# fluhus/frackyfrac

Measured on NVIDIA B200. Metric: UniFrac sample-pairs/sec (unweighted), higher is better.
Workload: dtype u8 x u8 -> s32 (tcgen05 kind::i8, exact), s64 chunk / row sums, f32 ratio / output

## Files before the change

### frackyfrac_b200/csrc/embed.cu

```cuda
#include "frc_internal.h"

namespace frc {

namespace {

constexpr int kThreads = 256;

__global__ void k_scatter_f64(const int64_t* __restrict__ row_ptr, const int32_t* __restrict__ col,
                              const double* __restrict__ val, int64_t s_base, int64_t s_end, double* E,
                              int64_t ld, int32_t* __restrict__ K, int32_t kp) {
  int64_t s = s_base + ((static_cast<int64_t>(blockIdx.x) * blockDim.x + threadIdx.x) >> 5);
  int lane = threadIdx.x & 31;
  if (s >= s_end) return;
  int64_t b = row_ptr[s], e = row_ptr[s + 1];
  for (int64_t k = b + lane; k < e; k += 32) {
    E[static_cast<int64_t>(col[k]) * ld + (s - s_base)] = val[k];
    if (K) K[((s >> 7) * kp + col[k]) * 128 + (s & 127)] = col[k];
  }
}

__global__ void k_level_sum_f64(const int32_t* __restrict__ nodes, const int32_t* __restrict__ child_ptr,
                                const int32_t* __restrict__ child_idx, double* E, int64_t ld,
                                int32_t* __restrict__ K, int32_t kp, int64_t s_base) {
  int32_t v = nodes[blockIdx.x];
// ... 170 lines not shown
  const int32_t v0 = blockIdx.x * 64;
  const int32_t w0 = blockIdx.y * 8;
  for (int idx = threadIdx.x; idx < 512; idx += 256) {
    int node = idx >> 3, word = idx & 7;
    uint32_t x = 0;
    if (v0 + node < n_nodes && w0 + word < nw)
      x = bits[static_cast<int64_t>(v0 + node) * nw + w0 + word];
    words[node][word] = x;
  }
  __syncthreads();
  const int wi = threadIdx.x >> 5, lane = threadIdx.x & 31;
  const int32_t va = v0 + 2 * lane, vb = va + 1;
  const uint32_t wa = words[2 * lane][wi], wb = words[2 * lane + 1][wi];
  const uint32_t ha = va < n_nodes ? len_hi[va] : 0, hb = vb < n_nodes ? len_hi[vb] : 0;
  const uint32_t la = va < n_nodes ? len_lo[va] : 0, lb = vb < n_nodes ? len_lo[vb] : 0;
  const int64_t s0 = (static_cast<int64_t>(w0) + wi) * 32;
#pragma unroll 4
  for (int it = 0; it < 32; ++it) {
    const int64_t s = s0 + it;
    if (s >= np) break;
    const uint32_t ba = (wa >> it) & 1u, bb = (wb >> it) & 1u;
    const int64_t o = s * kp + va;
    const uint32_t ma = 0u - ba, mb = 0u - bb;
    *reinterpret_cast<uint32_t*>(P + o) = (0x3F80u & ma) | ((0x3F80u & mb) << 16);
    *reinterpret_cast<uint32_t*>(Bh + o) = (ha & ma) | ((hb & mb) << 16);
    *reinterpret_cast<uint32_t*>(Bl + o) = (la & ma) | ((lb & mb) << 16);
  }
}


template <bool kSmem>
__global__ void __launch_bounds__(512)
k_embed_presence_fused(const int64_t* __restrict__ row_ptr, const int32_t* __restrict__ col,
                       int64_t n_samples, const int32_t* __restrict__ level_nodes,
                       const int32_t* __restrict__ level_parent, const int32_t* __restrict__ level_ptr,
                       int32_t height, int32_t n_nodes, int32_t kp, const int32_t* __restrict__ order,
                       uint32_t* __restrict__ node_scratch, uint32_t* __restrict__ bitsT, int32_t w0,
                       uint32_t* __restrict__ bitsS, const PeerPtrs peers) {
  extern __shared__ __align__(16) uint32_t smem_words[];
  __shared__ int32_t lptr[128];
  const int w = blockIdx.x + w0;
  const int tid = threadIdx.x, lane = tid & 31, warp = tid >> 5;
  uint32_t* colw = kSmem ? smem_words : node_scratch + static_cast<int64_t>(blockIdx.x) * n_nodes;

  for (int32_t v = tid; v < n_nodes; v += 512) colw[v] = 0u;
  if (tid < 128 && tid <= height + 1) lptr[tid] = level_ptr[tid];
  __syncthreads();
  {
    int64_t rb[2], re[2];
#pragma unroll
    for (int u = 0; u < 2; ++u) {
      const int64_t s = static_cast<int64_t>(w) * 32 + warp + 16 * u;
      rb[u] = s < n_samples ? row_ptr[s] : 0;
      re[u] = s < n_samples ? row_ptr[s + 1] : 0;
    }
#pragma unroll
    for (int u = 0; u < 2; ++u) {
      const uint32_t bit = 1u << (warp + 16 * u);
      for (int64_t k = rb[u] + lane; k < re[u]; k += 256) {
        int32_t c[8];
#pragma unroll
        for (int x = 0; x < 8; ++x) c[x] = k + 32 * x < re[u] ? col[k + 32 * x] : -1;
#pragma unroll
        for (int x = 0; x < 8; ++x)
          if (c[x] >= 0) atomicOr(colw + c[x], bit);
      }
    }
  }
  __syncthreads();
  auto lp = [&](int32_t h) { return h < 128 ? lptr[h] : level_ptr[h]; };
  int32_t h = 0;
  for (; h < height; ++h) {
    const int32_t b = lp(h), e = lp(h + 1);
    if (e - b <= 512) break;
    for (int32_t idx = b + tid; idx < e; idx += 4096) {
      int32_t n[8], p[8];
#pragma unroll
      for (int u = 0; u < 8; ++u) {
        const int32_t k = idx + u * 512;
        n[u] = k < e ? level_nodes[k] : -1;
        p[u] = k < e ? level_parent[k] : 0;
      }
#pragma unroll
      for (int u = 0; u < 8; ++u)
        if (n[u] >= 0) {
          const uint32_t x = colw[n[u]];
          if (x) atomicOr(colw + p[u], x);
        }
    }
    __syncthreads();
  }
  for (; h < height; h += 8) {
    int32_t n[8], p[8];
#pragma unroll
    for (int u = 0; u < 8; ++u) {
      n[u] = -1; p[u] = 0;
      if (h + u < height) {
        const int32_t k = lp(h + u) + tid;
        if (k < lp(h + u + 1)) { n[u] = level_nodes[k]; p[u] = level_parent[k]; }
      }
    }
#pragma unroll
    for (int u = 0; u < 8; ++u) {
      if (h + u < height) {
        if (n[u] >= 0) {
          const uint32_t x = colw[n[u]];
          if (x) atomicOr(colw + p[u], x);
        }
        __syncthreads();
      }
    }
  }
  uint32_t* dst = bitsT + static_cast<int64_t>(w) * kp;
  if (peers.n > 0) {
    const int64_t at = static_cast<int64_t>(w) * kp;
#pragma unroll 4
    for (int32_t k = tid; k < kp; k += 512) {
      const int32_t v = order[k];
      const uint32_t x = v >= 0 ? colw[v] : 0u;
#pragma unroll
      for (int pr = 0; pr < 8; ++pr)
        if (pr < peers.n) peers.p[pr][at + k] = x;
    }
  } else {
#pragma unroll 8
    for (int32_t k = tid; k < kp; k += 512) {
      const int32_t v = order[k];
      dst[k] = v >= 0 ? colw[v] : 0u;
    }
  }
  if (bitsS != nullptr) {
    const int32_t words = kp >> 5;
    for (int32_t g = warp; g * 128 < kp; g += 16) {
      uint32_t wout[4];
#pragma unroll
      for (int u = 0; u < 4; ++u) {
        const int32_t v = order[g * 128 + u * 32 + lane];
        const uint32_t wv = v >= 0 ? colw[v] : 0u;
        uint32_t mine = 0;
// ... 318 lines not shown
    ++launches;
  }
  return launches;
}

int launch_presence_rowsum(const uint32_t* bits, int32_t n_nodes, int32_t nw, const double* lenq,
                           double* r, double* scratch, cudaStream_t s) {
  int chunks = pick_chunks(n_nodes);
  dim3 grid(nw, chunks);
  k_presence_rowsum<<<grid, 32, 0, s>>>(bits, n_nodes, nw, lenq, scratch);
  int64_t ld = static_cast<int64_t>(nw) * 32;
  k_reduce_partials<<<static_cast<unsigned>((ld + kThreads - 1) / kThreads), kThreads, 0, s>>>(
      scratch, chunks, ld, ld, r);
  return 2;
}

int launch_expand_operands(const uint32_t* bits, int32_t n_nodes, int32_t nw, int32_t kp, int64_t np,
                           const uint16_t* len_hi, const uint16_t* len_lo, uint16_t* P, uint16_t* Bh,
                           uint16_t* Bl, cudaStream_t s) {
  dim3 grid(kp / 64, static_cast<unsigned>((np + 255) / 256));
  k_expand_operands<<<grid, 256, 0, s>>>(bits, n_nodes, nw, kp, np, len_hi, len_lo, P, Bh, Bl);
  return 1;
}


void embed_setup() {
  cudaFuncSetAttribute(k_embed_presence_fused<true>, cudaFuncAttributeMaxDynamicSharedMemorySize, 200 * 1024);
}

int64_t presence_node_scratch_words(int32_t n_nodes, int32_t nw) {
  return static_cast<size_t>(n_nodes) * 4 <= 200 * 1024 ? 0 : static_cast<int64_t>(n_nodes) * nw;
}

int launch_embed_presence_fused(const DevTree& t, const int32_t* level_ptr_dev, const DevCsr& a,
                                int32_t nw, int32_t w0, int32_t w_count, int32_t kp, const int32_t* order,
                                uint32_t* node_scratch, uint32_t* bitsT, uint32_t* bitsS, const PeerPtrs& peers,
                                cudaStream_t s) {
  (void)nw;
  const size_t smem = (static_cast<size_t>(t.n_nodes) * 4 + 15) & ~size_t(15);
  if (smem <= 200 * 1024) {
    k_embed_presence_fused<true><<<w_count, 512, smem, s>>>(a.row_ptr, a.col, a.n_samples, t.level_nodes,
                                                            t.level_parent, level_ptr_dev, t.height, t.n_nodes, kp,
                                                            order, node_scratch, bitsT, w0, bitsS, peers);
  } else {
    k_embed_presence_fused<false><<<w_count, 512, 0, s>>>(a.row_ptr, a.col, a.n_samples, t.level_nodes,
                                                          t.level_parent, level_ptr_dev, t.height, t.n_nodes, kp,
                                                          order, node_scratch, bitsT, w0, bitsS, peers);
  }
  return 1;
}

int launch_presence_rowsum_t(const uint32_t* bitsT, int32_t n_nodes, int32_t nw, int32_t w0, int32_t w_count,
                             int32_t kp, const double* lenq, const uint32_t* qam, const int32_t* col_exp,
                             double* partial, double* r, int32_t e_min, long long* r_int, cudaStream_t s) {
  const int64_t np = static_cast<int64_t>(nw) * 32;
  const int chunks = pick_chunks(n_nodes);
  dim3 g(w_count, chunks);
  const int64_t s0 = static_cast<int64_t>(w0) * 32, ns = static_cast<int64_t>(w_count) * 32;
  if (qam) {
    const int32_t per = static_cast<int32_t>(round_up((kp + chunks - 1) / chunks, 128));
    if (r_int) cudaMemsetAsync(r_int + s0, 0, sizeof(long long) * ns, s);
    k_presence_rowsum_u8<<<g, 32, 0, s>>>(bitsT, kp, per, qam, col_exp, partial, np, w0, e_min, r_int);
    if (r_int) return 1;
  } else {
    const int32_t per = static_cast<int32_t>(round_up((kp + chunks - 1) / chunks, 8));
    k_presence_rowsum_t<<<g, 32, 0, s>>>(bitsT, kp, per, lenq, partial, np, w0);
  }
  k_reduce_partials<<<static_cast<unsigned>((ns + kThreads - 1) / kThreads), kThreads, 0, s>>>(partial + s0, chunks, np,
                                                                                              ns, r + s0);
  return 2;
}

int launch_expand_operands_t(const uint32_t* bitsT, int32_t nw, int32_t kp, int64_t np, bool i8,
                             const void* q0, const void* q1, const void* q2, void* P, void* Bh, void* Bl,
                             const uint8_t* need, const uint32_t* qam, const int32_t* col_exp, int32_t e_min,
                             long long* r_int, cudaStream_t s) {
  if (i8) {
    if (r_int) cudaMemsetAsync(r_int, 0, sizeof(long long) * np, s);
    dim3 grid(kp / 128, static_cast<unsigned>((np + 255) / 256));
    k_expand_operands_u8<<<grid, 256, 0, s>>>(bitsT, nw, kp, np, static_cast<const uint8_t*>(q0),
                                              static_cast<const uint8_t*>(q1), static_cast<const uint8_t*>(q2),
                                              static_cast<uint8_t*>(P), static_cast<uint8_t*>(Bh),
                                              static_cast<uint8_t*>(Bl), need, qam, col_exp, e_min, r_int);
  } else {
    (void)q0;
    dim3 grid(kp / 64, static_cast<unsigned>((np + 255) / 256));
    k_expand_operands_t<<<grid, 256, 0, s>>>(bitsT, nw, kp, np, static_cast<const uint16_t*>(q1),
                                             static_cast<const uint16_t*>(q2), static_cast<uint16_t*>(P),
                                             static_cast<uint16_t*>(Bh), static_cast<uint16_t*>(Bl), need);
  }
  return 1;
}

int launch_quantize_lengths(const double* len_col, const int32_t* col_exp, int32_t kp, uint8_t* qa,
                            uint8_t* qh, uint8_t* ql, uint32_t* qam, double* lenq, double* qerr, double* flag_u,
                            cudaStream_t s) {
  k_quantize_lengths<<<(kp + 127) / 128, 128, 0, s>>>(len_col, col_exp, kp, qa, qh, ql, qam, lenq, qerr);
  k_sum_flag_u<<<1, 1024, 0, s>>>(qerr, kp, flag_u);
  return 2;
}

}
```

### frackyfrac_b200/csrc/frc_internal.h

```cpp
#pragma once
#include <cuda_runtime.h>
#include <cstdint>
#include <string>

namespace frc {

constexpr int kTile = 128;
constexpr int kKBlock = 64;

inline int64_t round_up(int64_t x, int64_t m) { return (x + m - 1) / m * m; }
inline int64_t tri(int64_t i) { return i * (i - 1) / 2; }

struct DevTree {
  int32_t n_nodes = 0;
  int32_t height = 0;
  const int32_t* parent = nullptr;
  const double* length = nullptr;
  const int32_t* child_ptr = nullptr;
  const int32_t* child_idx = nullptr;
  const int32_t* level_nodes = nullptr;
  const int32_t* level_parent = nullptr;
};

struct DevCsr {
// ... 15 lines not shown
struct Exceptions {
  unsigned long long* count = nullptr;
  int64_t* index = nullptr;
  double* value = nullptr;
  int32_t cap = 0;
};

int launch_embed_f64(const DevTree& t, const int32_t* level_ptr_host, const DevCsr& a, double* E,
                     int64_t ld, int64_t s_base, cudaStream_t s, int32_t* K = nullptr, int32_t kp = 0);
int launch_totals_f64(const double* E, int32_t n_nodes, int64_t ld, int64_t n_samples,
                      double* total, cudaStream_t s);
int launch_totals_fast_f64(const double* E, int32_t n_nodes, int64_t ld, const double* mult, double* total,
                           double* scratch, cudaStream_t s);
int launch_normalize_f64(double* E, int32_t n_nodes, int64_t ld, int64_t n_samples,
                         const double* total, cudaStream_t s);
int launch_weighted_operand(const double* E, const double* length, int32_t n_nodes, int32_t kp,
                            int64_t ld, int64_t n_samples, const double* total, bool prescale,
                            float* A, double* W, double* scratch, cudaStream_t s);
int launch_weighted_operand_panels(const double* E, const double* length, int32_t n_nodes, int32_t kp,
                                   int64_t ld, int64_t s_base, const double* total, bool prescale, float* Ap,
                                   double* W, double* scratch, cudaStream_t s);
int weighted_scratch_chunks(int32_t n_nodes);

int launch_embed_bits(const DevTree& t, const int32_t* level_ptr_host, const DevCsr& a,
                      uint32_t* bits, int32_t nw, cudaStream_t s);
int launch_presence_rowsum(const uint32_t* bits, int32_t n_nodes, int32_t nw, const double* lenq,
                           double* r, double* scratch, cudaStream_t s);
int launch_expand_operands(const uint32_t* bits, int32_t n_nodes, int32_t nw, int32_t kp,
                           int64_t np, const uint16_t* len_hi, const uint16_t* len_lo,
                           uint16_t* P, uint16_t* Bh, uint16_t* Bl, cudaStream_t s);

int64_t presence_node_scratch_words(int32_t n_nodes, int32_t nw);
void embed_setup();
int launch_embed_presence_fused(const DevTree& t, const int32_t* level_ptr_dev, const DevCsr& a,
                                int32_t nw, int32_t w0, int32_t w_count, int32_t kp, const int32_t* order,
                                uint32_t* node_scratch, uint32_t* bitsT, uint32_t* bitsS, const PeerPtrs& peers,
                                cudaStream_t s);
int launch_presence_rowsum_t(const uint32_t* bitsT, int32_t n_nodes, int32_t nw, int32_t w0, int32_t w_count,
                             int32_t kp, const double* lenq, const uint32_t* qam, const int32_t* col_exp,
                             double* partial, double* r, int32_t e_min, long long* r_int, cudaStream_t s);
int launch_expand_operands_t(const uint32_t* bitsT, int32_t nw, int32_t kp, int64_t np, bool i8,
                             const void* q0, const void* q1, const void* q2, void* P, void* Bh, void* Bl,
                             const uint8_t* need, const uint32_t* qam, const int32_t* col_exp, int32_t e_min,
                             long long* r_int, cudaStream_t s);
int launch_quantize_lengths(const double* len_col, const int32_t* col_exp, int32_t kp, uint8_t* qa,
                            uint8_t* qh, uint8_t* ql, uint32_t* qam, double* lenq, double* qerr, double* flag_u,
                            cudaStream_t s);

struct Comm;
bool comm_unique_id(char* id128, std::string* err);
Comm* comm_create(const char* id128, int rank, int world, std::string* err);
void comm_destroy(Comm* c);
int comm_rank(const Comm* c);
int comm_world(const Comm* c);
bool comm_all_gather_inplace(Comm* c, void* const* bufs, const size_t* bytes_per_rank, int n, cudaStream_t s,
                             std::string* err);

bool comm_all_gather_host(Comm* c, const void* mine, size_t bytes, void* all, cudaStream_t s, std::string* err);
bool comm_barrier(Comm* c, cudaStream_t s, std::string* err);

int launch_exact_pairs(const double* E, const double* length, int32_t n_nodes, int64_t ld,
                       bool weighted, int64_t first, int64_t count, double* out, cudaStream_t s);
int launch_postorder_lists(const double* E, const int32_t* post_order, int32_t n_nodes, int64_t ld, int64_t n_samples,
                           int64_t* list_ptr, int32_t* list_id, double* list_val, cudaStream_t s);
int launch_unsorted_pairs(const int64_t* list_ptr, const int32_t* list_id, const double* list_val,
                          const double* length, int64_t first, int64_t count, double* out, cudaStream_t s);

void widen_band(const float* src, double* dst, int64_t n, bool stream_stores);

// ... 44 lines not shown
```

### frackyfrac_b200/csrc/job.cu

```cuda
#include <algorithm>
#include <atomic>
#include <chrono>
#include <climits>
#include <cmath>
#include <cstdio>
#include <cstdlib>
#include <cstring>
#include <functional>
#include <memory>
#include <string>
#include <thread>
#include <vector>

#if defined(__x86_64__)
#include <immintrin.h>
#endif

#include "../../include/frcfrc_cuda.h"
#include "frc_internal.h"
#include "host_pool.h"
#include "plan.h"

using namespace frc;
using frc_host::Pool;
// ... 461 lines not shown
        if (norm) launches += launch_totals_fast_f64(p->d_E, sh.B, ld, p->d_mult, p->d_total + sb, p->d_scratch, s);
        launches += launch_weighted_operand_panels(p->d_E, p->dtree.length, sh.B, sh.kp, ld, sb,
                                                   norm ? p->d_total + sb : nullptr, sh.prescale, Ap, p->d_W,
                                                   p->d_scratch, s);
      }
      if (exchange_shard(p, arrs, rg, s)) return p->rc;
    }
    p->pm = PanelMap{};
    if (sh.capacity) {
      p->pm.n_shards = sh.shards.n_shards;
      p->pm.tiles_per_shard = static_cast<int32_t>(sh.shards.shard_rows / kTile);
      for (int k = 0; k < sh.shards.n_shards; ++k)
        if (sh.shards.owner[k] == p->owner) p->pm.shard[k] = p->d_A + sh.shards.slot[k] * sh.shards.shard_rows * sh.kp;
    } else {
      p->pm.shard[0] = p->d_A;
    }
    p->info.embed_bytes = 2LL * sh.B * built * (sh.keyed ? 12 : 8) + 12LL * (p->csr_k1 - p->csr_k0);
  } else if (sh.fused_embed) {
    const int cur = static_cast<int>(p->run_count & 1);
    if (p->peer_push) {
      p->d_bits = p->d_bits2[cur];
      if (p->run_count == 0) {
        std::string cerr;
        if (!comm_barrier(c->comm, s, &cerr)) return pfail(p, FRC_ERR_CUDA, cerr);
      }
    }
    ++p->run_count;
    PeerPtrs peers;
    if (p->peer_push) peers = p->peers[cur];
    else if (inproc && !sh.bits_feed) {
      peers.n = sh.n_parts; peers.self = p->index;
      for (int q = 0; q < sh.n_parts; ++q) peers.p[q] = p->job->parts[q]->d_bits;
    }
    launches += launch_embed_presence_fused(p->dtree, p->d_level_ptr, p->dcsr, sh.nw, p->shard_w0, p->shard_nw,
                                            sh.kp, p->d_order, p->d_node_scratch, p->d_bits, p->d_bitsS, peers, s);
    const bool rowsum_in_expand = sh.cols.intacc && !sh.bits_feed;
    const bool split = sh.exchange == Shared::kNone && !rowsum_in_expand;
    cudaStream_t rs = split ? dc->stream[1] : s;
    if (split) {
      PART_CUDA(p, cudaEventRecord(p->ev_bits, s));
      PART_CUDA(p, cudaStreamWaitEvent(rs, p->ev_bits, 0));
    }
    if (!rowsum_in_expand)
      launches += launch_presence_rowsum_t(p->d_bits, sh.B, sh.nw, p->shard_w0, p->shard_nw, sh.kp, p->d_lenq,
                                           sh.cols.i8 ? p->d_qam : nullptr, p->d_col_exp, p->d_scratch, p->d_r,
                                           sh.cols.e_min, sh.cols.intacc ? p->d_r_int : nullptr, rs);
    std::vector<ShardArray> arrs;
    if (!rowsum_in_expand)
      arrs.push_back({sh.cols.intacc ? part_array<&Part::d_r_int> : part_array<&Part::d_r>, sizeof(double)});
    arrs.push_back({sh.bits_feed ? part_array<&Part::d_bitsS> : part_array<&Part::d_bits>, sizeof(uint32_t) * sh.kp / 32,
                    peers.n == 0});
    if (exchange_shard(p, arrs, sh.shards.ranges[p->owner][0], s)) return p->rc;
    if (sh.exchange != Shared::kNone) {
      p->info.embed_bytes = 2LL * sh.B * p->shard_nw * 4 + 4LL * (p->csr_k1 - p->csr_k0);
    }
  }
  PART_CUDA(p, cudaGetLastError());
  if (inproc) PART_CUDA(p, cudaEventRecord(p->ev_shard, s));
  p->info.kernel_launches += launches;
  return FRC_OK;
}

int embed_stage2(Part* p) {
  const Shared& sh = *p->sh;
  DevCtx* dc = p->dc;
  cudaStream_t s = dc->stream[0];
  int launches = 0;
  if (sh.exchange == Shared::kInProcess)
    for (auto& o : p->job->parts)
// ... 499 lines not shown
                                          "panels of all samples on every device; the capacity mode, which shards them "
                                          "over the devices when they exceed about half of one device's free HBM (or with "
                                          "FRC_CAPACITY=1), does not carry keys");
    sh.capacity = want;
    if (want) mode = ShardPlan::kCapacity;
  }
  sh.shards = plan_shards(sh.N, owners, mode);
  sh.np = sh.shards.np;
  sh.nw = static_cast<int32_t>(sh.np / 32);
  sh.kp = static_cast<int32_t>(round_up(sh.B, kKBlock));
  sh.prescale = !neg_len;
  if (fast_uw) {
    const bool want_i8 = sh.fused_embed && !neg_len && !(sh.opts.flags & FRC_FLAG_UW_BF16) && !sh.knobs.uw_bf16;
    sh.cols = plan_columns(tree->length, sh.B, want_i8, sh.knobs.group_binades, sh.knobs.u8_acc_f64, tc_chunk_kblocks());
    sh.kp = sh.cols.kp;
    sh.bits_feed = sh.cols.intacc && ((sh.opts.flags & FRC_FLAG_UW_BITS) != 0 || sh.knobs.feed_bits);
    if (sh.cols.intacc && !sh.bits_feed) {
      const double need = 3.0 * static_cast<double>(sh.np) * sh.kp;
      if (need > 32.0 * (1 << 30)) {
        size_t free_b = 0, total_b = 0;
        cudaSetDevice(c->devs[0]->device);
        if (cudaMemGetInfo(&free_b, &total_b) == cudaSuccess && need > 0.80 * static_cast<double>(free_b)) sh.bits_feed = true;
        cudaGetLastError();
      }
    }
  }
  sh.bands = sh.capacity ? make_bands_capacity(sh.N, sh.shards, sh.opts.band_rows, sh.d2h)
                         : make_bands(sh.N, sh.opts.band_rows, owners, sh.d2h, sh.knobs.bands_per_rank, 8);
  for (const Band& b : sh.bands)
    if (b.count >= (1LL << 32)) return fail(j, FRC_ERR_UNSUPPORTED, "band too large; lower band_rows");
  return FRC_OK;
}

int stage_plan(frc_job* j, const frc_tree_t* tree) {
  Shared& sh = j->sh;
  const ColumnPlan& cp = sh.cols;
  SegAlloc seg;
  sh.pl_q0 = seg(sh.kp); sh.pl_hi = seg(sizeof(uint16_t) * sh.kp); sh.pl_lo = seg(sizeof(uint16_t) * sh.kp);
  sh.pl_lenq = seg(sizeof(double) * sh.kp);
  sh.pl_order = seg(sizeof(int32_t) * cp.col_order.size()); sh.pl_cexp = seg(sizeof(int32_t) * cp.col_exp.size());
  sh.pl_lcol = seg(sizeof(double) * cp.len_col.size()); sh.pl_cend = seg(sizeof(int32_t) * cp.chunk_end.size());
  sh.pl_cscale = seg(sizeof(double) * cp.chunk_scale.size()); sh.pl_cshift = seg(sizeof(int32_t) * cp.chunk_shift.size());
  sh.plan_bytes = seg.total;
  cudaError_t e = cudaSuccess;
  sh.stage_plan = static_cast<char*>(j->ctx->pin.alloc(sh.plan_bytes, &e));
  if (!sh.stage_plan) return fail(j, FRC_ERR_OOM, std::string("pinned staging: ") + cudaGetErrorString(e));
  char* st = sh.stage_plan;
  if (!sh.exact && !sh.weighted && !cp.i8) {
    uint16_t* hi = reinterpret_cast<uint16_t*>(st + sh.pl_hi.off);
    uint16_t* lo = reinterpret_cast<uint16_t*>(st + sh.pl_lo.off);
    double* lq = reinterpret_cast<double*>(st + sh.pl_lenq.off);
    for (int32_t v = 0; v < sh.B; ++v) {
      const double l = tree->length[v];
      hi[v] = bf16_rn(static_cast<float>(l));
      const double res = l - static_cast<double>(bf16_to_float(hi[v]));
      lo[v] = (l == l && !std::isinf(l)) ? bf16_rn(static_cast<float>(res)) : 0;
      lq[v] = static_cast<double>(bf16_to_float(hi[v])) + static_cast<double>(bf16_to_float(lo[v]));
    }
    for (int32_t v = sh.B; v < sh.kp; ++v) { hi[v] = 0; lo[v] = 0; lq[v] = 0.0; }
  }
  auto put = [&](const Seg& s, const void* src) { if (s.bytes) memcpy(st + s.off, src, s.bytes); };
  put(sh.pl_order, cp.col_order.data()); put(sh.pl_cexp, cp.col_exp.data()); put(sh.pl_lcol, cp.len_col.data());
  put(sh.pl_cend, cp.chunk_end.data()); put(sh.pl_cscale, cp.chunk_scale.data()); put(sh.pl_cshift, cp.chunk_shift.data());
  return FRC_OK;
}

int prepare_part(Part* p) {
  const Shared& sh = *p->sh;
  DevCtx* dc = p->dc;
  frc_ctx* c = p->job->ctx;
  const int32_t B = sh.B;
  PART_CUDA(p, cudaSetDevice(dc->device));
  p->max_band = 1;
  for (size_t k = 0; k < sh.bands.size(); ++k)
    if (sh.bands[k].owner == p->owner) {
      p->mine.push_back(static_cast<int>(k));
      p->bands.push_back(sh.bands[k]);
      p->info.n_pairs_mine += sh.bands[k].count;
      p->max_band = std::max(p->max_band, sh.bands[k].count);
    }
  const bool fast_uw = !sh.exact && !sh.weighted;
  if (sh.capacity) {
    const std::vector<CapGroupPlan> groups =
        plan_capacity_groups(p->bands, sh.N, sh.shards.shard_rows, sh.shards.n_shards, p->tiles, p->band_group);
    for (const CapGroupPlan& gp : groups) {
      if (gp.count >= (1LL << 32)) return pfail(p, FRC_ERR_UNSUPPORTED, "capacity mode: a row shard holds 2^32 pairs or more");
      Part::CapGroup g;
      g.shard = gp.shard; g.first = gp.first; g.count = gp.count; g.tile_off = gp.tile_off; g.coff = gp.coff;
      p->cap.push_back(g);
    }
  } else if (!sh.exact) {
    for (Band& b : p->bands) append_band_tiles(b, fast_uw, p->tiles);
  }
  std::vector<uint8_t> need;
  if (fast_uw && sh.shards.ranges.size() > 1 && sh.fused_embed) need = operand_need_blocks(p->tiles, sh.np, true);
// ... 307 lines not shown
    j->parts.emplace_back(new Part());
    Part* p = j->parts.back().get();
    p->job = j; p->sh = &sh; p->dc = c->devs[k]; p->index = k;
    p->owner = sh.n_parts > 1 ? k : sh.rank0;
  }

  const frc_tree_t* const tree0 = tree;
  PrunedTree pruned;
  frc_tree_t ptree{};
  if (opts->flags & FRC_FLAG_PRUNE) {
    std::vector<int32_t> depth(B0);
    int32_t bad_parent = 0, bad_order = 0;
    if (check_preorder(tree0->parent, B0, depth.data(), &bad_parent, &bad_order)) {
      std::vector<uint8_t> marks(B0, 0);
      const int T = nnz >= 65536 ? c->pool->size() : 1;
      const std::function<void(int)> mark_leaves = [&](int t) {
        const int64_t k1 = nnz * (t + 1) / T;
        for (int64_t k = nnz * t / T; k < k1; ++k) {
          const int32_t cc = abnd->col[k];
          if (cc >= 0 && cc < B0 && !__atomic_load_n(&marks[cc], __ATOMIC_RELAXED))
            __atomic_store_n(&marks[cc], uint8_t{1}, __ATOMIC_RELAXED);
        }
      };
      c->pool->run(T, mark_leaves);
      pruned = prune_tree(tree0->parent, tree0->length, B0, marks.data(), !sh.exact);
      ptree = frc_tree_t{pruned.n_nodes, pruned.parent.data(), pruned.length.data()};
      tree = &ptree;
      sh.B = pruned.n_nodes;
      sh.node_mult = !sh.exact && sh.weighted && opts->normalize == 1;
    }
  }
  const int32_t B = sh.B;
  const int32_t* const new_of_old = pruned.new_of_old.empty() ? nullptr : pruned.new_of_old.data();

  layout_inputs(sh);
  {
    cudaError_t e = cudaSuccess;
    sh.stage_in = static_cast<char*>(c->pin.alloc(sh.in_bytes, &e));
    if (!sh.stage_in) return bail(fail(j, FRC_ERR_OOM, std::string("pinned staging of the inputs: ") + cudaGetErrorString(e)));
    int64_t* rp = reinterpret_cast<int64_t*>(sh.stage_in + sh.in_rowptr.off);
    if (N > 0) memcpy(rp, abnd->row_ptr, sizeof(int64_t) * (N + 1)); else rp[0] = 0;
  }
  char* const stage_in = sh.stage_in;

  TreeLevels levels;
  bool children_ok = false;
  std::atomic<int> plan_ready{0};
  auto tree_children_share = [&]() {
    if (!tree_children(tree->parent, B, reinterpret_cast<int32_t*>(stage_in + sh.in_cptr.off),
                       reinterpret_cast<int32_t*>(stage_in + sh.in_cidx.off))) return;
    memcpy(stage_in + sh.in_parent.off, tree->parent, sizeof(int32_t) * B);
    memcpy(stage_in + sh.in_len.off, tree->length, sizeof(double) * B);
    float* lf = reinterpret_cast<float*>(stage_in + sh.in_lenf.off);
    const int32_t kp_pad = static_cast<int32_t>(round_up(B, kKBlock));
    for (int32_t v = 0; v < kp_pad; ++v) lf[v] = v < B ? static_cast<float>(tree->length[v]) : 0.f;
    if (sh.unsorted_l) tree_post_order(tree->parent, B, reinterpret_cast<int32_t*>(stage_in + sh.in_post.off));
    if (sh.node_mult) {
      double* m = reinterpret_cast<double*>(stage_in + sh.in_mult.off);
      for (int32_t v = 0; v < B; ++v) m[v] = pruned.mult[v];
    }
    children_ok = true;
  };
  auto tree_levels_share = [&]() {
    levels = tree_levels(tree->parent, B, reinterpret_cast<int32_t*>(stage_in + sh.in_lvl.off),
                         reinterpret_cast<int32_t*>(stage_in + sh.in_lpar.off));
    if (levels.height >= 0)
      memcpy(stage_in + sh.in_lptr.off, levels.level_ptr.data(), sizeof(int32_t) * (levels.height + 2));
  };
  int64_t stage_k0 = 0, stage_k1 = nnz;
  const int csr_chunks = nnz >= 65536 ? static_cast<int>(std::max<int64_t>(1, std::min<int64_t>(c->pool->size() * 8LL, nnz / 8192))) : 1;
  const int n_prep = sh.n_parts - 1;
  const int n_tasks = 2 + n_prep + csr_chunks;
  std::atomic<int> task_next{0};
  std::vector<std::string> csr_errs(csr_chunks);
  std::vector<double> csr_us(c->pool->size(), 0.0);
  const int64_t stamp_tag = c->stamp_epoch;
  c->stamp_epoch += N + 1;
  const std::function<void(int)> work = [&](int t) {
    const auto w0 = std::chrono::steady_clock::now();
    int32_t* dcol = reinterpret_cast<int32_t*>(stage_in + sh.in_col.off);
    double* dval = sh.need_val ? reinterpret_cast<double*>(stage_in + sh.in_val.off) : nullptr;
    const int TS = csr_chunks;
    const bool check_dup = sh.need_val;
    const int32_t* parent = tree0->parent;
    auto row_at = [&](int64_t target) {
      return static_cast<int64_t>(std::lower_bound(abnd->row_ptr, abnd->row_ptr + N, target) - abnd->row_ptr);
    };
    std::vector<int64_t>& stamp = c->stamps[t];
    if (check_dup && static_cast<int32_t>(stamp.size()) < B0) stamp.assign(B0, -1);
    for (int task = task_next.fetch_add(1, std::memory_order_relaxed); task < n_tasks;
         task = task_next.fetch_add(1, std::memory_order_relaxed)) {
      if (task == 0) { tree_levels_share(); continue; }
      if (task == 1) { tree_children_share(); continue; }
      if (task < 2 + n_prep) {
        int ready;
        while ((ready = plan_ready.load(std::memory_order_acquire)) == 0) std::this_thread::yield();
        if (ready > 0) prepare_part(j->parts[task - 1].get());
        continue;
      }
      const int ch = task - 2 - n_prep;
      const int64_t span = stage_k1 - stage_k0;
      const int64_t s0 = row_at(stage_k0 + span * ch / TS), s1 = ch == TS - 1 ? row_at(stage_k1) : row_at(stage_k0 + span * (ch + 1) / TS);
      bool failed = false;
      for (int64_t s = s0; s < s1 && !failed; ++s) {
        const int64_t b = abnd->row_ptr[s], e = abnd->row_ptr[s + 1];
        const int64_t mark_s = stamp_tag + s;
        for (int64_t k = b; k < e; ++k) {
          const int32_t cc = abnd->col[k];
          const double v = abnd->val[k];
          const char* what = nullptr;
          if (cc < 0 || cc >= B0) what = "node id out of range";
          else if (cc + 1 < B0 && parent[cc + 1] == cc) what = "node is not a leaf";
          else if (!(v > 0) || std::isinf(v)) what = "bad value";
          else if (check_dup && stamp[cc] == mark_s) what = "leaf listed twice";
          if (what) {
            csr_errs[ch] = "sample #" + std::to_string(s + 1) + ": entry " + std::to_string(k - b + 1) + " (node " +
                           std::to_string(cc) + "): " + what;
            failed = true;
            break;
          }
          if (check_dup) stamp[cc] = mark_s;
          const int32_t id = new_of_old ? new_of_old[cc] : cc;
#if defined(__x86_64__)
          _mm_stream_si32(dcol + k, id);
          if (dval) _mm_stream_si64(reinterpret_cast<long long*>(dval + k), static_cast<long long>(__builtin_bit_cast(int64_t, v)));
#else
          dcol[k] = id;
          if (dval) dval[k] = v;
#endif
        }
      }
    }
#if defined(__x86_64__)
    _mm_sfence();
#endif
    csr_us[t] += std::chrono::duration<double, std::micro>(std::chrono::steady_clock::now() - w0).count();
  };
  if (!sh.exact && !sh.weighted && sh.n_parts == 1 && sh.world > 1 && (opts->flags & FRC_FLAG_SHARD_EMBED) && N > 0) {
    const Range own = plan_shards(N, sh.world, ShardPlan::kSharded).ranges[sh.rank0][0];
    stage_k0 = abnd->row_ptr[std::min(N, own.s0)]; stage_k1 = abnd->row_ptr[std::min(N, own.s1)];
  }
  const int n_workers = c->pool->size() - 1;
  if (n_workers > 0) {
    workers_busy = true;
    c->pool->start(n_workers, work);
  }
  mark("header checks, context, workers started");

  bool neg_len = false, bad_len = false;
  for (int32_t v = 0; v < B0; ++v) {
    const double l = tree0->length[v];
    if (!(l == l) || std::isinf(l)) bad_len = true;
  }
  for (int32_t v = 0; v < B; ++v) {
    const double l = tree->length[v];
    if (l < 0 && !std::isinf(l)) neg_len = true;
  }
  auto plan_failed = [&](int code) { plan_ready.store(-1, std::memory_order_release); return bail(code); };
  if (!sh.exact && bad_len)
    return plan_failed(fail(j, FRC_ERR_UNSUPPORTED, "non-finite branch length: only the exact path handles it"));
  if ((rc = plan_job(j, tree, neg_len)) != FRC_OK) return plan_failed(rc);
  if ((rc = stage_plan(j, tree)) != FRC_OK) return plan_failed(rc);
  mark("column plan + bands");
  plan_ready.store(1, std::memory_order_release);
  prepare_part(j->parts[0].get());
  mark("device 0 prepared");
  work(n_workers);
  if (workers_busy) { c->pool->wait(); workers_busy = false; }
  if (trace) { fprintf(stderr, "[frc_create] share times (us):"); for (double u : csr_us) fprintf(stderr, " %.0f", u); fprintf(stderr, "\n"); }
  if (levels.bad_parent) return bail(fail(j, FRC_ERR_ARG, "parent[" + std::to_string(levels.bad_parent) + "] is not a smaller node id"));
  if (levels.bad_order) return bail(fail(j, FRC_ERR_ARG, "node ids are not a pre-order numbering (node " + std::to_string(levels.bad_order) + ")"));
  for (auto& e : csr_errs)
    if (!e.empty()) return bail(fail(j, FRC_ERR_ARG, e));
  if (levels.height < 0 || !children_ok) return bail(fail(j, FRC_ERR_ARG, "tree topology could not be prepared"));
  for (auto& p : j->parts)
    if (p->rc) { j->err = p->err; return bail(p->rc); }
  sh.level_ptr = levels.level_ptr;
  sh.tree_height = levels.height;
  {
    std::vector<int> cursor(sh.n_parts, 0);
    for (const Band& b : sh.bands)
      for (int k = 0; k < sh.n_parts; ++k)
        if (j->parts[k]->owner == b.owner) { j->order.push_back({k, cursor[k]++}); break; }
  }
  if (!sh.exact && sh.d2h) {
    int64_t mb = 1;
    for (auto& p : j->parts) mb = std::max(mb, p->max_band);
    cudaError_t e = cudaSuccess;
    j->wide = static_cast<double*>(c->pin.alloc(sizeof(double) * std::min(mb, kWidePiece), &e));
    if (!j->wide) return bail(fail(j, FRC_ERR_OOM, std::string("pinned widening buffer: ") + cudaGetErrorString(e)));
  }
  mark("workers joined");
  if ((rc = for_parts(j, launch_part_stage1)) != FRC_OK) return bail(rc);
  if ((rc = for_parts(j, launch_part_stage2)) != FRC_OK) return bail(rc);
  mark("uploads, embedding, first bands queued");
// ... 240 lines not shown
```

### frackyfrac_b200/csrc/plan.cpp

```cpp
#include "plan.h"

#include <algorithm>
#include <climits>
#include <cmath>
#include <cstring>

namespace frc {

static std::vector<int> band_owners_lpt(const std::vector<int64_t>& rows, int world) {
  const size_t n = rows.size() > 0 ? rows.size() - 1 : 0;
  std::vector<int> owner(n, 0);
  std::vector<size_t> order(n);
  std::vector<int64_t> cnt(n);
  for (size_t k = 0; k < n; ++k) {
    order[k] = k;
    cnt[k] = tri(rows[k + 1]) - (rows[k] >= 2 ? tri(rows[k]) : 0);
  }
  std::stable_sort(order.begin(), order.end(), [&](size_t a, size_t b) { return cnt[a] > cnt[b]; });
  std::vector<int64_t> load(world, 0);
  for (size_t k : order) {
    int best = 0;
    for (int r = 1; r < world; ++r)
      if (load[r] < load[best]) best = r;
    owner[k] = best;
// ... 276 lines not shown
    for (int32_t c = 0; c < pairw; ++c)
      if ((static_cast<int64_t>(t.tj) + c) * kTile < np) need[(t.tj + c) / 2] |= 1;
  }
  return need;
}

bool check_preorder(const int32_t* parent, int32_t B, int32_t* depth, int32_t* bad_parent, int32_t* bad_order) {
  *bad_parent = 0; *bad_order = 0;
  std::vector<int32_t> on_path(B + 1, 0);
  depth[0] = 0;
  for (int32_t v = 1; v < B; ++v) {
    const int32_t p = parent[v];
    if (p < 0 || p >= v) { *bad_parent = v; return false; }
    const int32_t d = depth[p];
    if ((d > depth[v - 1] || on_path[d] != p) && !*bad_order) *bad_order = v;
    depth[v] = d + 1;
    on_path[d + 1] = v;
  }
  return !*bad_order;
}

TreeLevels tree_levels(const int32_t* parent, int32_t B, int32_t* lvl, int32_t* lpar) {
  TreeLevels out;
  std::vector<int32_t> depth(B, 0), height(B, 0);
  if (!check_preorder(parent, B, depth.data(), &out.bad_parent, &out.bad_order)) return out;
  for (int32_t v = B - 1; v >= 1; --v) height[parent[v]] = std::max(height[parent[v]], height[v] + 1);
  const int32_t H = height[0];
  out.level_ptr.assign(H + 2, 0);
  for (int32_t v = 0; v < B; ++v) out.level_ptr[height[v] + 1]++;
  for (int32_t h = 0; h <= H; ++h) out.level_ptr[h + 1] += out.level_ptr[h];
  std::vector<int32_t>& lfill = depth;
  for (int32_t h = 0; h <= H; ++h) lfill[h] = out.level_ptr[h];
  for (int32_t v = 0; v < B; ++v) lvl[lfill[height[v]]++] = v;
  for (int32_t k = 0; k < B; ++k) lpar[k] = lvl[k] ? parent[lvl[k]] : 0;
  out.height = H;
  return out;
}

bool tree_children(const int32_t* parent, int32_t B, int32_t* cptr, int32_t* cidx) {
  std::vector<int32_t> child_cnt(B, 0);
  for (int32_t v = 1; v < B; ++v) {
    const int32_t p = parent[v];
    if (p < 0 || p >= v) return false;
    child_cnt[p]++;
  }
  cptr[0] = 0;
  for (int32_t v = 0; v < B; ++v) cptr[v + 1] = cptr[v] + child_cnt[v];
  std::vector<int32_t>& fill = child_cnt;
  for (int32_t v = 0; v < B; ++v) fill[v] = cptr[v];
  for (int32_t v = 1; v < B; ++v) cidx[fill[parent[v]]++] = v;
  return true;
}

void tree_post_order(const int32_t* parent, int32_t B, int32_t* post_order) {
  std::vector<int32_t> size(B, 1), depth(B, 0);
  for (int32_t v = B - 1; v >= 1; --v) size[parent[v]] += size[v];
  for (int32_t v = 1; v < B; ++v) depth[v] = depth[parent[v]] + 1;
  for (int32_t v = 0; v < B; ++v) post_order[v + size[v] - 1 - depth[v]] = v;
}

PrunedTree prune_tree(const int32_t* parent, const double* length, int32_t B, const uint8_t* marks, bool merge) {
  std::vector<uint8_t> keep(B);
  std::vector<int32_t> kids(B, 0);
  for (int32_t v = 0; v < B; ++v) keep[v] = marks[v] ? 1 : 0;
  if (B > 0) keep[0] = 1;
  for (int32_t v = B - 1; v >= 1; --v)
    if (keep[v]) { keep[parent[v]] = 1; kids[parent[v]]++; }
  if (merge)
    for (int32_t v = 1; v < B; ++v)
// ... 85 lines not shown
int64_t frc_debug_band_tiles(int64_t row0, int64_t row1, int32_t pair_tiles, int32_t* out2, int64_t cap) {
  frc::Band b;
  b.row0 = row0; b.row1 = row1;
  std::vector<frc::Tile> tiles;
  frc::append_band_tiles(b, pair_tiles != 0, tiles);
  for (size_t k = 0; k < tiles.size() && static_cast<int64_t>(k) < cap; ++k) { out2[2 * k] = tiles[k].ti; out2[2 * k + 1] = tiles[k].tj; }
  return static_cast<int64_t>(tiles.size());
}

int32_t frc_debug_plan_columns(const double* length, int32_t n_nodes, int32_t want_i8, int32_t group_binades,
                               int32_t force_f64, int32_t* col_order, int32_t* col_exp, double* len_col, int32_t cap,
                               int32_t* chunk_end, double* chunk_scale, int32_t* chunk_shift, int32_t* info) {
  const frc::ColumnPlan p = frc::plan_columns(length, n_nodes, want_i8 != 0, group_binades, force_f64 != 0, 64);
  if (p.kp > cap || p.chunk_end.size() > 64) return -p.kp;
  for (int32_t k = 0; k < p.kp; ++k) {
    col_order[k] = p.col_order[k];
    col_exp[k] = p.col_exp.empty() ? 0 : p.col_exp[k];
    len_col[k] = p.len_col[k];
  }
  for (size_t c = 0; c < p.chunk_end.size(); ++c) {
    chunk_end[c] = p.chunk_end[c];
    chunk_scale[c] = p.chunk_scale[c];
    chunk_shift[c] = p.chunk_shift.empty() ? 0 : p.chunk_shift[c];
  }
  info[0] = p.i8; info[1] = p.intacc; info[2] = p.biased; info[3] = p.e_min; info[4] = static_cast<int32_t>(p.chunk_end.size());
  return p.kp;
}

int32_t frc_debug_tree(const int32_t* parent, int32_t n_nodes, int32_t* level_nodes, int32_t* level_parent,
                       int32_t* level_ptr, int32_t* child_ptr, int32_t* child_idx, int32_t* post_order) {
  const frc::TreeLevels t = frc::tree_levels(parent, n_nodes, level_nodes, level_parent);
  if (t.bad_parent) return -1 - t.bad_parent;
  if (t.bad_order) return -1 - t.bad_order;
  for (size_t k = 0; k < t.level_ptr.size(); ++k) level_ptr[k] = t.level_ptr[k];
  if (!frc::tree_children(parent, n_nodes, child_ptr, child_idx)) return -1;
  frc::tree_post_order(parent, n_nodes, post_order);
  return t.height;
}

int32_t frc_debug_prune(const int32_t* parent, const double* length, int32_t n_nodes, const uint8_t* marks, int32_t merge,
                        int32_t* out_parent, double* out_length, int32_t* out_mult, int32_t* new_of_old) {
  std::vector<int32_t> depth(n_nodes);
  int32_t bad_parent = 0, bad_order = 0;
  if (!frc::check_preorder(parent, n_nodes, depth.data(), &bad_parent, &bad_order)) return -1 - (bad_parent ? bad_parent : bad_order);
  const frc::PrunedTree t = frc::prune_tree(parent, length, n_nodes, marks, merge != 0);
  for (int32_t v = 0; v < t.n_nodes; ++v) { out_parent[v] = t.parent[v]; out_length[v] = t.length[v]; out_mult[v] = t.mult[v]; }
  for (int32_t v = 0; v < n_nodes; ++v) new_of_old[v] = t.new_of_old[v];
  return t.n_nodes;
}

}
```

### frackyfrac_b200/csrc/plan.h

```cpp
#pragma once
#include <cstdint>
#include <string>
#include <vector>

#include "frc_internal.h"

namespace frc {

struct Band {
  int64_t row0 = 0, row1 = 0;
  int64_t first = 0, count = 0;
  int32_t tile_off = 0, n_tiles = 0;
  int owner = 0;
};

std::vector<int64_t> band_boundaries(int64_t N, int64_t requested, int world, bool d2h, int per_rank, int value_bytes);
std::vector<int> band_owners(const std::vector<int64_t>& rows, int world);
std::vector<Band> make_bands(int64_t N, int64_t requested, int world, bool d2h, int per_rank, int value_bytes);

struct Range { int64_t s0, s1, slot; };
struct ShardPlan {
  enum Mode { kWhole, kSharded, kCapacity };
  int64_t np = 0, shard_rows = 0;
  int n_shards = 1;
// ... 6 lines not shown

struct CapGroupPlan {
  int shard = 0;
  int64_t first = 0, count = 0;
  int32_t tile_off = 0;
  std::vector<int32_t> coff;
};
std::vector<CapGroupPlan> plan_capacity_groups(const std::vector<Band>& bands, int64_t N, int64_t shard_rows, int n_shards,
                                               std::vector<Tile>& tiles, std::vector<int>& band_group);

struct ColumnPlan {
  bool i8 = false;
  bool intacc = false;
  bool biased = false;
  int32_t kp = 0;
  int32_t e_min = 0;
  std::vector<int32_t> col_order;
  std::vector<int32_t> col_exp;
  std::vector<double> len_col;
  std::vector<int32_t> chunk_end;
  std::vector<double> chunk_scale;
  std::vector<int32_t> chunk_shift;
};
ColumnPlan plan_columns(const double* length, int32_t n_nodes, bool want_i8, int group_binades, bool force_f64_acc,
                        int bf16_chunk_kblocks);

void append_band_tiles(Band& b, bool pair_tiles, std::vector<Tile>& tiles);
std::vector<uint8_t> operand_need_blocks(const std::vector<Tile>& tiles, int64_t np, bool pair_tiles);

struct TreeLevels {
  int32_t height = -1;
  int32_t bad_parent = 0, bad_order = 0;
  std::vector<int32_t> level_ptr;
};
bool check_preorder(const int32_t* parent, int32_t n_nodes, int32_t* depth, int32_t* bad_parent, int32_t* bad_order);
TreeLevels tree_levels(const int32_t* parent, int32_t n_nodes, int32_t* level_nodes, int32_t* level_parent);
bool tree_children(const int32_t* parent, int32_t n_nodes, int32_t* child_ptr, int32_t* child_idx);
void tree_post_order(const int32_t* parent, int32_t n_nodes, int32_t* post_order);

struct PrunedTree {
  int32_t n_nodes = 0;
  std::vector<int32_t> parent, new_of_old;
  std::vector<double> length;
  std::vector<int32_t> mult;
};
PrunedTree prune_tree(const int32_t* parent, const double* length, int32_t n_nodes, const uint8_t* marks, bool merge);

}
```

Measured before the change: 30.99 billion.

## Renumber tree nodes in level order so presence embed skips node indirection

Node ids are remapped on the host into level-order positions: leaf columns in the staged CSR, the column order and level_parent all use these positions. The presence-embed kernel can then read colw directly by level index instead of going through level_nodes. Parent indices for the first level are prefetched into registers ahead of each level's synchronisation, and the separate r_int memset is folded into the embed kernel. The cost is extra host-side mapping work, a wait on the tree-level computation before staging the plan, and a changed meaning of level_parent that every consumer must agree with.

```diff
diff --git a/frackyfrac_b200/csrc/embed.cu b/frackyfrac_b200/csrc/embed.cu
--- a/frackyfrac_b200/csrc/embed.cu
+++ b/frackyfrac_b200/csrc/embed.cu
@@ -226,19 +226,31 @@
 template <bool kSmem>
 __global__ void __launch_bounds__(512)
 k_embed_presence_fused(const int64_t* __restrict__ row_ptr, const int32_t* __restrict__ col,
-                       int64_t n_samples, const int32_t* __restrict__ level_nodes,
-                       const int32_t* __restrict__ level_parent, const int32_t* __restrict__ level_ptr,
-                       int32_t height, int32_t n_nodes, int32_t kp, const int32_t* __restrict__ order,
-                       uint32_t* __restrict__ node_scratch, uint32_t* __restrict__ bitsT, int32_t w0,
-                       uint32_t* __restrict__ bitsS, const PeerPtrs peers) {
+                       int64_t n_samples, const int32_t* __restrict__ level_parent,
+                       const int32_t* __restrict__ level_ptr, int32_t height, int32_t n_nodes, int32_t kp,
+                       const int32_t* __restrict__ order, uint32_t* __restrict__ node_scratch,
+                       uint32_t* __restrict__ bitsT, int32_t w0, uint32_t* __restrict__ bitsS, const PeerPtrs peers,
+                       long long* __restrict__ r_int, int64_t np) {
   extern __shared__ __align__(16) uint32_t smem_words[];
   __shared__ int32_t lptr[128];
   const int w = blockIdx.x + w0;
   const int tid = threadIdx.x, lane = tid & 31, warp = tid >> 5;
   uint32_t* colw = kSmem ? smem_words : node_scratch + static_cast<int64_t>(blockIdx.x) * n_nodes;
 
+  int32_t pf[8];
+  {
+    const int32_t e0 = level_ptr[1];
+#pragma unroll
+    for (int u = 0; u < 8; ++u) {
+      const int32_t k = tid + u * 512;
+      pf[u] = k < e0 ? level_parent[k] : 0;
+    }
+  }
   for (int32_t v = tid; v < n_nodes; v += 512) colw[v] = 0u;
   if (tid < 128 && tid <= height + 1) lptr[tid] = level_ptr[tid];
+  if (r_int != nullptr)
+    for (int64_t i = static_cast<int64_t>(blockIdx.x) * 512 + tid; i < np; i += static_cast<int64_t>(gridDim.x) * 512)
+      r_int[i] = 0;
   __syncthreads();
   {
     int64_t rb[2], re[2];
@@ -267,38 +279,56 @@
   for (; h < height; ++h) {
     const int32_t b = lp(h), e = lp(h + 1);
     if (e - b <= 512) break;
-    for (int32_t idx = b + tid; idx < e; idx += 4096) {
-      int32_t n[8], p[8];
+#pragma unroll
+    for (int u = 0; u < 8; ++u) {
+      const int32_t k = b + tid + u * 512;
+      if (k < e) {
+        const uint32_t x = colw[k];
+        if (x) atomicOr(colw + pf[u], x);
+      }
+    }
+    for (int32_t idx = b + 4096 + tid; idx < e; idx += 4096) {
+      int32_t p[8];
 #pragma unroll
       for (int u = 0; u < 8; ++u) {
         const int32_t k = idx + u * 512;
-        n[u] = k < e ? level_nodes[k] : -1;
         p[u] = k < e ? level_parent[k] : 0;
       }
 #pragma unroll
       for (int u = 0; u < 8; ++u)
-        if (n[u] >= 0) {
-          const uint32_t x = colw[n[u]];
+        if (idx + u * 512 < e) {
+          const uint32_t x = colw[idx + u * 512];
           if (x) atomicOr(colw + p[u], x);
         }
     }
+    if (h + 1 < height) {
+      const int32_t e1 = lp(h + 2);
+#pragma unroll
+      for (int u = 0; u < 8; ++u) {
+        const int32_t k = e + tid + u * 512;
+        pf[u] = k < e1 ? level_parent[k] : 0;
+      }
+    }
     __syncthreads();
   }
   for (; h < height; h += 8) {
-    int32_t n[8], p[8];
+    int32_t k[8], p[8];
 #pragma unroll
     for (int u = 0; u < 8; ++u) {
-      n[u] = -1; p[u] = 0;
+      k[u] = -1; p[u] = 0;
       if (h + u < height) {
-        const int32_t k = lp(h + u) + tid;
-        if (k < lp(h + u + 1)) { n[u] = level_nodes[k]; p[u] = level_parent[k]; }
+        const int32_t kk = lp(h + u) + tid;
+        if (kk < lp(h + u + 1)) {
+          k[u] = kk;
+          p[u] = level_parent[kk];
+        }
       }
     }
 #pragma unroll
     for (int u = 0; u < 8; ++u) {
       if (h + u < height) {
-        if (n[u] >= 0) {
-          const uint32_t x = colw[n[u]];
+        if (k[u] >= 0) {
+          const uint32_t x = colw[k[u]];
           if (x) atomicOr(colw + p[u], x);
         }
         __syncthreads();
@@ -683,21 +713,19 @@
   return static_cast<size_t>(n_nodes) * 4 <= 200 * 1024 ? 0 : static_cast<int64_t>(n_nodes) * nw;
 }
 
-int launch_embed_presence_fused(const DevTree& t, const int32_t* level_ptr_dev, const DevCsr& a,
-                                int32_t nw, int32_t w0, int32_t w_count, int32_t kp, const int32_t* order,
-                                uint32_t* node_scratch, uint32_t* bitsT, uint32_t* bitsS, const PeerPtrs& peers,
+int launch_embed_presence_fused(const DevTree& t, const int32_t* level_ptr_dev, const DevCsr& a, int32_t w0,
+                                int32_t w_count, int32_t kp, const int32_t* order, uint32_t* node_scratch,
+                                uint32_t* bitsT, uint32_t* bitsS, const PeerPtrs& peers, long long* r_int, int64_t np,
                                 cudaStream_t s) {
-  (void)nw;
   const size_t smem = (static_cast<size_t>(t.n_nodes) * 4 + 15) & ~size_t(15);
-  if (smem <= 200 * 1024) {
-    k_embed_presence_fused<true><<<w_count, 512, smem, s>>>(a.row_ptr, a.col, a.n_samples, t.level_nodes,
-                                                            t.level_parent, level_ptr_dev, t.height, t.n_nodes, kp,
-                                                            order, node_scratch, bitsT, w0, bitsS, peers);
-  } else {
-    k_embed_presence_fused<false><<<w_count, 512, 0, s>>>(a.row_ptr, a.col, a.n_samples, t.level_nodes,
-                                                          t.level_parent, level_ptr_dev, t.height, t.n_nodes, kp,
-                                                          order, node_scratch, bitsT, w0, bitsS, peers);
-  }
+  if (smem <= 200 * 1024)
+    k_embed_presence_fused<true><<<w_count, 512, smem, s>>>(a.row_ptr, a.col, a.n_samples, t.level_parent, level_ptr_dev,
+                                                            t.height, t.n_nodes, kp, order, node_scratch, bitsT, w0,
+                                                            bitsS, peers, r_int, np);
+  else
+    k_embed_presence_fused<false><<<w_count, 512, 0, s>>>(a.row_ptr, a.col, a.n_samples, t.level_parent, level_ptr_dev,
+                                                          t.height, t.n_nodes, kp, order, node_scratch, bitsT, w0,
+                                                          bitsS, peers, r_int, np);
   return 1;
 }
 
@@ -727,7 +755,6 @@
                              const uint8_t* need, const uint32_t* qam, const int32_t* col_exp, int32_t e_min,
                              long long* r_int, cudaStream_t s) {
   if (i8) {
-    if (r_int) cudaMemsetAsync(r_int, 0, sizeof(long long) * np, s);
     dim3 grid(kp / 128, static_cast<unsigned>((np + 255) / 256));
     k_expand_operands_u8<<<grid, 256, 0, s>>>(bitsT, nw, kp, np, static_cast<const uint8_t*>(q0),
                                               static_cast<const uint8_t*>(q1), static_cast<const uint8_t*>(q2),
diff --git a/frackyfrac_b200/csrc/frc_internal.h b/frackyfrac_b200/csrc/frc_internal.h
--- a/frackyfrac_b200/csrc/frc_internal.h
+++ b/frackyfrac_b200/csrc/frc_internal.h
@@ -71,9 +71,9 @@
 
 int64_t presence_node_scratch_words(int32_t n_nodes, int32_t nw);
 void embed_setup();
-int launch_embed_presence_fused(const DevTree& t, const int32_t* level_ptr_dev, const DevCsr& a,
-                                int32_t nw, int32_t w0, int32_t w_count, int32_t kp, const int32_t* order,
-                                uint32_t* node_scratch, uint32_t* bitsT, uint32_t* bitsS, const PeerPtrs& peers,
+int launch_embed_presence_fused(const DevTree& t, const int32_t* level_ptr_dev, const DevCsr& a, int32_t w0,
+                                int32_t w_count, int32_t kp, const int32_t* order, uint32_t* node_scratch,
+                                uint32_t* bitsT, uint32_t* bitsS, const PeerPtrs& peers, long long* r_int, int64_t np,
                                 cudaStream_t s);
 int launch_presence_rowsum_t(const uint32_t* bitsT, int32_t n_nodes, int32_t nw, int32_t w0, int32_t w_count,
                              int32_t kp, const double* lenq, const uint32_t* qam, const int32_t* col_exp,
diff --git a/frackyfrac_b200/csrc/job.cu b/frackyfrac_b200/csrc/job.cu
--- a/frackyfrac_b200/csrc/job.cu
+++ b/frackyfrac_b200/csrc/job.cu
@@ -517,9 +517,10 @@
       peers.n = sh.n_parts; peers.self = p->index;
       for (int q = 0; q < sh.n_parts; ++q) peers.p[q] = p->job->parts[q]->d_bits;
     }
-    launches += launch_embed_presence_fused(p->dtree, p->d_level_ptr, p->dcsr, sh.nw, p->shard_w0, p->shard_nw,
-                                            sh.kp, p->d_order, p->d_node_scratch, p->d_bits, p->d_bitsS, peers, s);
     const bool rowsum_in_expand = sh.cols.intacc && !sh.bits_feed;
+    launches += launch_embed_presence_fused(p->dtree, p->d_level_ptr, p->dcsr, p->shard_w0, p->shard_nw, sh.kp,
+                                            p->d_order, p->d_node_scratch, p->d_bits, p->d_bitsS, peers,
+                                            rowsum_in_expand ? p->d_r_int : nullptr, sh.np, s);
     const bool split = sh.exchange == Shared::kNone && !rowsum_in_expand;
     cudaStream_t rs = split ? dc->stream[1] : s;
     if (split) {
@@ -1085,7 +1086,7 @@
   return FRC_OK;
 }
 
-int stage_plan(frc_job* j, const frc_tree_t* tree) {
+int stage_plan(frc_job* j, const frc_tree_t* tree, const int32_t* node_pos) {
   Shared& sh = j->sh;
   const ColumnPlan& cp = sh.cols;
   SegAlloc seg;
@@ -1114,6 +1115,10 @@
   }
   auto put = [&](const Seg& s, const void* src) { if (s.bytes) memcpy(st + s.off, src, s.bytes); };
   put(sh.pl_order, cp.col_order.data()); put(sh.pl_cexp, cp.col_exp.data()); put(sh.pl_lcol, cp.len_col.data());
+  if (node_pos) {
+    int32_t* order = reinterpret_cast<int32_t*>(st + sh.pl_order.off);
+    for (size_t k = 0; k < cp.col_order.size(); ++k) order[k] = cp.col_order[k] >= 0 ? node_pos[cp.col_order[k]] : -1;
+  }
   put(sh.pl_cend, cp.chunk_end.data()); put(sh.pl_cscale, cp.chunk_scale.data()); put(sh.pl_cshift, cp.chunk_shift.data());
   return FRC_OK;
 }
@@ -1487,6 +1492,19 @@
   }
   const int32_t B = sh.B;
   const int32_t* const new_of_old = pruned.new_of_old.empty() ? nullptr : pruned.new_of_old.data();
+  const bool stage_positions = !sh.exact && !sh.weighted && !sh.knobs.embed_levels;
+  std::vector<int32_t> stage_map;
+  if (stage_positions) {
+    std::vector<int32_t> lpos(B);
+    leaf_positions(tree->parent, B, lpos.data());
+    if (new_of_old) {
+      stage_map.resize(B0);
+      for (int32_t v = 0; v < B0; ++v) stage_map[v] = new_of_old[v] >= 0 ? lpos[new_of_old[v]] : -1;
+    } else {
+      stage_map = std::move(lpos);
+    }
+  }
+  const int32_t* const id_map = stage_positions ? stage_map.data() : new_of_old;
 
   layout_inputs(sh);
   {
@@ -1499,6 +1517,7 @@
   char* const stage_in = sh.stage_in;
 
   TreeLevels levels;
+  std::atomic<int> levels_done{0};
   bool children_ok = false;
   std::atomic<int> plan_ready{0};
   auto tree_children_share = [&]() {
@@ -1521,6 +1540,7 @@
                          reinterpret_cast<int32_t*>(stage_in + sh.in_lpar.off));
     if (levels.height >= 0)
       memcpy(stage_in + sh.in_lptr.off, levels.level_ptr.data(), sizeof(int32_t) * (levels.height + 2));
+    levels_done.store(1, std::memory_order_release);
   };
   int64_t stage_k0 = 0, stage_k1 = nnz;
   const int csr_chunks = nnz >= 65536 ? static_cast<int>(std::max<int64_t>(1, std::min<int64_t>(c->pool->size() * 8LL, nnz / 8192))) : 1;
@@ -1575,7 +1595,7 @@
             break;
           }
           if (check_dup) stamp[cc] = mark_s;
-          const int32_t id = new_of_old ? new_of_old[cc] : cc;
+          const int32_t id = id_map ? id_map[cc] : cc;
 #if defined(__x86_64__)
           _mm_stream_si32(dcol + k, id);
           if (dval) _mm_stream_si64(reinterpret_cast<long long*>(dval + k), static_cast<long long>(__builtin_bit_cast(int64_t, v)));
@@ -1615,7 +1635,13 @@
   if (!sh.exact && bad_len)
     return plan_failed(fail(j, FRC_ERR_UNSUPPORTED, "non-finite branch length: only the exact path handles it"));
   if ((rc = plan_job(j, tree, neg_len)) != FRC_OK) return plan_failed(rc);
-  if ((rc = stage_plan(j, tree)) != FRC_OK) return plan_failed(rc);
+  if (stage_positions) {
+    int expected = 0;
+    if (task_next.compare_exchange_strong(expected, 1)) tree_levels_share();
+    while (!levels_done.load(std::memory_order_acquire)) std::this_thread::yield();
+  }
+  if ((rc = stage_plan(j, tree, stage_positions && levels.height >= 0 ? levels.pos.data() : nullptr)) != FRC_OK)
+    return plan_failed(rc);
   mark("column plan + bands");
   plan_ready.store(1, std::memory_order_release);
   prepare_part(j->parts[0].get());
diff --git a/frackyfrac_b200/csrc/plan.cpp b/frackyfrac_b200/csrc/plan.cpp
--- a/frackyfrac_b200/csrc/plan.cpp
+++ b/frackyfrac_b200/csrc/plan.cpp
@@ -332,9 +332,19 @@
   std::vector<int32_t>& lfill = depth;
   for (int32_t h = 0; h <= H; ++h) lfill[h] = out.level_ptr[h];
   for (int32_t v = 0; v < B; ++v) lvl[lfill[height[v]]++] = v;
-  for (int32_t k = 0; k < B; ++k) lpar[k] = lvl[k] ? parent[lvl[k]] : 0;
+  out.pos.resize(B);
+  for (int32_t k = 0; k < B; ++k) out.pos[lvl[k]] = k;
+  for (int32_t k = 0; k < B; ++k) lpar[k] = lvl[k] ? out.pos[parent[lvl[k]]] : 0;
   out.height = H;
   return out;
+}
+
+void leaf_positions(const int32_t* parent, int32_t B, int32_t* pos) {
+  int32_t n = 0;
+  for (int32_t v = 0; v < B; ++v) {
+    pos[v] = n;
+    n += v + 1 == B || parent[v + 1] != v;
+  }
 }
 
 bool tree_children(const int32_t* parent, int32_t B, int32_t* cptr, int32_t* cidx) {
@@ -486,6 +496,7 @@
   const frc::TreeLevels t = frc::tree_levels(parent, n_nodes, level_nodes, level_parent);
   if (t.bad_parent) return -1 - t.bad_parent;
   if (t.bad_order) return -1 - t.bad_order;
+  for (int32_t k = 0; k < n_nodes; ++k) level_parent[k] = level_nodes[k] ? level_nodes[level_parent[k]] : 0;
   for (size_t k = 0; k < t.level_ptr.size(); ++k) level_ptr[k] = t.level_ptr[k];
   if (!frc::tree_children(parent, n_nodes, child_ptr, child_idx)) return -1;
   frc::tree_post_order(parent, n_nodes, post_order);
diff --git a/frackyfrac_b200/csrc/plan.h b/frackyfrac_b200/csrc/plan.h
--- a/frackyfrac_b200/csrc/plan.h
+++ b/frackyfrac_b200/csrc/plan.h
@@ -62,9 +62,11 @@
   int32_t height = -1;
   int32_t bad_parent = 0, bad_order = 0;
   std::vector<int32_t> level_ptr;
+  std::vector<int32_t> pos;
 };
 bool check_preorder(const int32_t* parent, int32_t n_nodes, int32_t* depth, int32_t* bad_parent, int32_t* bad_order);
 TreeLevels tree_levels(const int32_t* parent, int32_t n_nodes, int32_t* level_nodes, int32_t* level_parent);
+void leaf_positions(const int32_t* parent, int32_t n_nodes, int32_t* pos);
 bool tree_children(const int32_t* parent, int32_t n_nodes, int32_t* child_ptr, int32_t* child_idx);
 void tree_post_order(const int32_t* parent, int32_t n_nodes, int32_t* post_order);
 
```

New measurement: 31.31 billion, median of 6. 1.01x the previous value.
